# yanqinJiang/Animate3D

Measured on NVIDIA H100. Metric: MV-VDM denoise-steps/sec @ 4view x 16frame x 256^2, higher is better.
Workload: dtype fp16

## Files before the change

### animate3d_b200/csrc/a3d_attn.cu

```cuda
#include <stdlib.h>

#include <type_traits>

#include "a3d_common.cuh"
#include "a3d_host.cuh"
#include "a3d_wgmma.cuh"

namespace a3d {

struct AttnDev {
  int q_tiles, kv_tiles;
  int rows_q, rows_k;
  int heads;
  int q_t1, q_box1, q_box2, q_e1, q_e3;
  int k_t1, k_box1, k_box2, k_e3, kv_div, kv_i3_zero;
  uint32_t q_box_bytes, k_box_bytes;
  float scale_log2;
  __half* out;
  int64_t os1, os2, os3, os4;
  int accumulate;
  float out_scale;
  unsigned long long* dbg;
};

constexpr float kRescaleLog2 = 8.0f;
constexpr int kAttnThreads = 288;

template <int D>
struct AttnCfg {
  static constexpr int kDqk = (D + 15) / 16 * 16;
  static constexpr int kDv = (D + 1 + 15) / 16 * 16;
  static constexpr int kQB = (kDqk + 63) / 64;
  static constexpr int kVB = (kDv + 63) / 64;
  static constexpr int kStages = (D == 160) ? 3 : 4;
  static constexpr int kQBox = 128 * 128;
  static constexpr int kKVBox = 64 * 128;
  static constexpr int kSmemQ = kQB * kQBox;
  static constexpr int kSmemK = kStages * kQB * kKVBox;
  static constexpr int kSmemV = kStages * kVB * kKVBox;
  static constexpr int kSmemBytes = kSmemQ + kSmemK + kSmemV + 1024 + 256;
  static constexpr int kMinBlocks = (kSmemBytes <= 113 * 1024) ? 2 : 1;
  static_assert(kSmemBytes <= 227 * 1024, "shared memory budget");
};

template <int I, int N, class F>
__device__ __forceinline__ void static_for(F&& f) {
  if constexpr (I < N) {
    if (f(std::integral_constant<int, I>{})) static_for<I + 1, N>(f);
  }
}

template <int N>
__device__ __forceinline__ void wgmma_pv(float (&o)[N / 2], const uint32_t (&a)[4], uint64_t bdesc, uint32_t acc) {
  if constexpr (N == 48) wgmma_rs_n48<1>(o, a, bdesc, acc);
  else if constexpr (N == 96) wgmma_rs_n96<1>(o, a, bdesc, acc);
  else wgmma_rs_n176<1>(o, a, bdesc, acc);
}

template <int D>
__global__ void __launch_bounds__(kAttnThreads, AttnCfg<D>::kMinBlocks)
attn_tc_kernel(const AttnDev p, const __grid_constant__ CUtensorMap mapQ, const __grid_constant__ CUtensorMap mapK,
               const __grid_constant__ CUtensorMap mapV) {
  using Cfg = AttnCfg<D>;
  constexpr int S = Cfg::kStages;
  extern __shared__ uint8_t smem_raw[];
  uint8_t* smem = reinterpret_cast<uint8_t*>((reinterpret_cast<uintptr_t>(smem_raw) + 1023) & ~uintptr_t(1023));
  uint8_t* sQ = smem;
  uint8_t* sK = sQ + Cfg::kSmemQ;
  uint8_t* sV = sK + Cfg::kSmemK;
  uint64_t* bars = reinterpret_cast<uint64_t*>(sV + Cfg::kSmemV);
  uint64_t* q_full = bars;
  uint64_t* k_full = bars + 1;
  uint64_t* v_full = k_full + S;
  uint64_t* kv_empty = v_full + S;

  const int warp = threadIdx.x >> 5;
  const int lane = threadIdx.x & 31;
  const int qt = blockIdx.x;
  const int head = blockIdx.y;
  const int qb = blockIdx.z;
  const int n = p.kv_tiles;
  const int rows_tile = p.k_box1 * p.k_box2;

  if (p.rows_q < 128 || rows_tile < 64) {
    uint4* z = reinterpret_cast<uint4*>(sQ);
    const int n16 = (Cfg::kSmemQ + Cfg::kSmemK + Cfg::kSmemV) / 16;
    for (int i = threadIdx.x; i < n16; i += blockDim.x) z[i] = make_uint4(0, 0, 0, 0);
    fence_proxy_async_smem();
  }
  if (warp == 8 && lane == 0) {
    tma_prefetch_desc(&mapQ);
    tma_prefetch_desc(&mapK);
    tma_prefetch_desc(&mapV);
    mbar_init(q_full, 1);
    for (int i = 0; i < S; ++i) {
      mbar_init(&k_full[i], 1);
      mbar_init(&v_full[i], 1);
      mbar_init(&kv_empty[i], 8);
    }
    mbar_fence_init();
  }
  __syncthreads();

  const int q_i1 = (qt % p.q_t1) * p.q_box1;
  const int q_i2 = (qt / p.q_t1) * p.q_box2;
  const int q_i3 = qb % p.q_e3;
  const int q_i4 = qb / p.q_e3;

  if (warp == 8) {
    if (lane == 0) {
      const int kb = qb / p.kv_div;
      const int k_i3 = p.kv_i3_zero ? 0 : (kb % p.k_e3);
      const int k_i4 = kb / p.k_e3;
      mbar_expect_tx(q_full, p.q_box_bytes * Cfg::kQB);
#pragma unroll
      for (int b = 0; b < Cfg::kQB; ++b)
        tma_load_5d(sQ + b * Cfg::kQBox, &mapQ, q_full, head * Cfg::kDqk + b * 64, q_i1, q_i2, q_i3, q_i4);
      for (int j = 0; j < n; ++j) {
        const int st = j % S;
        const int k_i1 = (j % p.k_t1) * p.k_box1, k_i2 = (j / p.k_t1) * p.k_box2;
        mbar_wait(&kv_empty[st], ((j / S) & 1) ^ 1);
        mbar_expect_tx(&k_full[st], p.k_box_bytes * Cfg::kQB);
#pragma unroll
        for (int b = 0; b < Cfg::kQB; ++b)
          tma_load_5d(sK + (st * Cfg::kQB + b) * Cfg::kKVBox, &mapK, &k_full[st], head * Cfg::kDqk + b * 64, k_i1, k_i2, k_i3,
                      k_i4);
        mbar_expect_tx(&v_full[st], p.k_box_bytes * Cfg::kVB);
#pragma unroll
        for (int b = 0; b < Cfg::kVB; ++b)
          tma_load_5d(sV + (st * Cfg::kVB + b) * Cfg::kKVBox, &mapV, &v_full[st], head * Cfg::kDv + b * 64, k_i1, k_i2, k_i3,
                      k_i4);
      }
    }
    return;
  }

  const int wg = warp >> 2;
  const int g = lane >> 2, t = lane & 3;
  float s[32];
  float o[Cfg::kDv / 2];
#pragma unroll
  for (int i = 0; i < Cfg::kDv / 2; ++i) o[i] = 0.f;
  float m_lo = -INFINITY, m_hi = -INFINITY;
  const uint64_t qdesc = make_smem_desc_sw128(smem_u32(sQ + wg * (64 * 128)), 16, 1024);
  const uint64_t kdesc = make_smem_desc_sw128(smem_u32(sK), 16, 1024);
  const uint64_t vdesc = make_smem_desc_sw128(smem_u32(sV), Cfg::kKVBox, 1024);
  const int mask_from = rows_tile < 64 ? 0 : n - 1;
  uint32_t ph = 0;
  mbar_wait(q_full, 0);
  for (int j0 = 0; j0 < n; j0 += S) {
    static_for<0, S>([&](auto stc) {
      constexpr int st = decltype(stc)::value;
      const int j = j0 + st;
      if (j >= n) return false;
      mbar_wait(&k_full[st], ph);
      wgmma_fence();
#pragma unroll
      for (int kk = 0; kk < Cfg::kDqk / 16; ++kk)
        wgmma_ss_n64<0>(s, desc_add(qdesc, (kk / 4) * Cfg::kQBox + (kk % 4) * 32),
                        desc_add(kdesc, (st * Cfg::kQB + kk / 4) * Cfg::kKVBox + (kk % 4) * 32), kk ? 1u : 0u);
      wgmma_commit();
      wgmma_wait<0>();
      reg_fence(s);
      if (j >= mask_from) {
        const int valid = (j == n - 1) ? p.rows_k : rows_tile;
#pragma unroll
        for (int jj = 0; jj < 8; ++jj) {
#pragma unroll
          for (int e = 0; e < 2; ++e)
            if (8 * jj + 2 * t + e >= valid) { s[4 * jj + e] = -INFINITY; s[4 * jj + 2 + e] = -INFINITY; }
        }
      }
      float mx_lo = -INFINITY, mx_hi = -INFINITY;
#pragma unroll
      for (int jj = 0; jj < 8; ++jj) {
#pragma unroll
        for (int e = 0; e < 2; ++e) {
          mx_lo = fmaxf(mx_lo, s[4 * jj + e]);
          mx_hi = fmaxf(mx_hi, s[4 * jj + 2 + e]);
        }
      }
#pragma unroll
      for (int x = 1; x <= 2; x <<= 1) {
        mx_lo = fmaxf(mx_lo, __shfl_xor_sync(0xffffffffu, mx_lo, x));
        mx_hi = fmaxf(mx_hi, __shfl_xor_sync(0xffffffffu, mx_hi, x));
      }
      const float mn_lo = fmaxf(m_lo, mx_lo * p.scale_log2), mn_hi = fmaxf(m_hi, mx_hi * p.scale_log2);
      if (st == 0 && j == 0) {
        m_lo = mn_lo; m_hi = mn_hi;
      } else if (__any_sync(0xffffffffu, mn_lo - m_lo > kRescaleLog2 || mn_hi - m_hi > kRescaleLog2)) {
        if (p.dbg && lane == 0) atomicAdd(p.dbg, 1ull);
        const float a_lo = ex2_approx(m_lo - mn_lo), a_hi = ex2_approx(m_hi - mn_hi);
#pragma unroll
        for (int c = 0; c < Cfg::kDv / 8; ++c) {
          o[4 * c] *= a_lo; o[4 * c + 1] *= a_lo; o[4 * c + 2] *= a_hi; o[4 * c + 3] *= a_hi;
        }
        m_lo = mn_lo; m_hi = mn_hi;
      }
      uint32_t pa[4][4];
#pragma unroll
      for (int kk = 0; kk < 4; ++kk) {
#pragma unroll
        for (int h = 0; h < 2; ++h) {
          const float* sb = s + 4 * (2 * kk + h);
          pa[kk][2 * h] = pack_f16x2(ex2_approx(fmaf(sb[0], p.scale_log2, -m_lo)), ex2_approx(fmaf(sb[1], p.scale_log2, -m_lo)));
          pa[kk][2 * h + 1] = pack_f16x2(ex2_approx(fmaf(sb[2], p.scale_log2, -m_hi)), ex2_approx(fmaf(sb[3], p.scale_log2, -m_hi)));
        }
      }
      mbar_wait(&v_full[st], ph);
      wgmma_fence();
#pragma unroll
      for (int kk = 0; kk < 4; ++kk)
        wgmma_pv<Cfg::kDv>(o, pa[kk], desc_add(vdesc, st * Cfg::kVB * Cfg::kKVBox + kk * 2048), 1u);
      wgmma_commit();
      wgmma_wait<0>();
      reg_fence(o);
      __syncwarp();
      if (lane == 0) mbar_arrive(&kv_empty[st]);
      return true;
    });
    ph ^= 1;
  }
  const float l_lo = __shfl_sync(0xffffffffu, o[4 * (D / 8)], lane & ~3);
  const float l_hi = __shfl_sync(0xffffffffu, o[4 * (D / 8) + 2], lane & ~3);
#pragma unroll
  for (int h = 0; h < 2; ++h) {
    const int r = wg * 64 + (warp & 3) * 16 + g + 8 * h;
    const int i1 = q_i1 + r % p.q_box1;
    if (r >= p.rows_q || i1 >= p.q_e1) continue;
    const float inv = p.out_scale / (h ? l_hi : l_lo);
    const int i2 = q_i2 + r / p.q_box1;
    __half* orow = p.out + (int64_t)i1 * p.os1 + (int64_t)i2 * p.os2 + (int64_t)q_i3 * p.os3 + (int64_t)q_i4 * p.os4 +
                   head * D + 2 * t;
#pragma unroll
    for (int c = 0; c < D / 8; ++c) {
      float v0 = o[4 * c + 2 * h] * inv, v1 = o[4 * c + 2 * h + 1] * inv;
      if (p.accumulate) {
        const float2 f = __half22float2(*reinterpret_cast<const __half2*>(orow + 8 * c));
        v0 += f.x; v1 += f.y;
      }
      *reinterpret_cast<uint32_t*>(orow + 8 * c) = pack_f16x2(v0, v1);
    }
  }
}

struct ViewDev {
  const __half* base;
  int64_t s1, s2, s3, s4;
  int e1, e2, e3, e4;
};

constexpr int kFewKeysMax = 8;

template <int D>
__global__ void __launch_bounds__(256)
attn_fewkeys_kernel(ViewDev q, ViewDev k, ViewDev v, __half* out, int64_t os1, int64_t os2, int64_t os3, int64_t os4, int heads,
                    int dqk, int dv, float scale_log2, int kv_div, int kv_i3_zero, int accumulate, float out_scale) {
  constexpr int d = D;
  const int Lq = q.e1 * q.e2, Lk = k.e1 * k.e2;
  const int64_t total = (int64_t)q.e3 * q.e4 * Lq * heads;
  const int64_t idx = (int64_t)blockIdx.x * blockDim.x + threadIdx.x;
  if (idx >= total) return;
  const int h = (int)(idx % heads);
  const int64_t row = idx / heads;
  const int l = (int)(row % Lq);
  const int qb = (int)(row / Lq);
  const int kb = qb / kv_div;
  const __half* qp = q.base + (int64_t)(l % q.e1) * q.s1 + (int64_t)(l / q.e1) * q.s2 + (int64_t)(qb % q.e3) * q.s3 +
                     (int64_t)(qb / q.e3) * q.s4 + h * dqk;
  const int64_t koff = (int64_t)(kv_i3_zero ? 0 : kb % k.e3) * k.s3 + (int64_t)(kb / k.e3) * k.s4 + h * dqk;
  const int64_t voff = (int64_t)(kv_i3_zero ? 0 : kb % v.e3) * v.s3 + (int64_t)(kb / v.e3) * v.s4 + h * dv;
  int64_t krow[kFewKeysMax], vrow[kFewKeysMax];
#pragma unroll
  for (int j = 0; j < kFewKeysMax; ++j) {
    const int jj = j < Lk ? j : 0;
    krow[j] = koff + (int64_t)(jj % k.e1) * k.s1 + (int64_t)(jj / k.e1) * k.s2;
    vrow[j] = voff + (int64_t)(jj % v.e1) * v.s1 + (int64_t)(jj / v.e1) * v.s2;
  }
  float sc[kFewKeysMax];
#pragma unroll
  for (int j = 0; j < kFewKeysMax; ++j) sc[j] = 0.f;
#pragma unroll
  for (int c = 0; c < d; c += 8) {
    const uint4 qv = *reinterpret_cast<const uint4*>(qp + c);
    const __half2* qh = reinterpret_cast<const __half2*>(&qv);
    float2 qf[4];
#pragma unroll
    for (int t = 0; t < 4; ++t) qf[t] = __half22float2(qh[t]);
#pragma unroll
    for (int j = 0; j < kFewKeysMax; ++j) {
      if (j < Lk) {
        const uint4 kv = __ldg(reinterpret_cast<const uint4*>(k.base + krow[j] + c));
        const __half2* kh = reinterpret_cast<const __half2*>(&kv);
#pragma unroll
        for (int t = 0; t < 4; ++t) {
          const float2 kf = __half22float2(kh[t]);
          sc[j] = fmaf(qf[t].x, kf.x, fmaf(qf[t].y, kf.y, sc[j]));
        }
      }
    }
  }
  float m = -INFINITY;
#pragma unroll
  for (int j = 0; j < kFewKeysMax; ++j)
    if (j < Lk) m = fmaxf(m, sc[j]);
  float sum = 0.f;
#pragma unroll
  for (int j = 0; j < kFewKeysMax; ++j) {
    sc[j] = j < Lk ? exp2f((sc[j] - m) * scale_log2) : 0.f;
    sum += sc[j];
  }
  const float inv = out_scale / sum;
  __half* op = out + (int64_t)(l % q.e1) * os1 + (int64_t)(l / q.e1) * os2 + (int64_t)(qb % q.e3) * os3 +
               (int64_t)(qb / q.e3) * os4 + h * d;
#pragma unroll
  for (int c = 0; c < d; c += 8) {
    float acc[8];
#pragma unroll
    for (int t = 0; t < 8; ++t) acc[t] = 0.f;
#pragma unroll
    for (int j = 0; j < kFewKeysMax; ++j) {
      if (j < Lk) {
        const uint4 vv = __ldg(reinterpret_cast<const uint4*>(v.base + vrow[j] + c));
        const __half2* vh = reinterpret_cast<const __half2*>(&vv);
#pragma unroll
        for (int t = 0; t < 4; ++t) {
          const float2 vf = __half22float2(vh[t]);
          acc[2 * t] = fmaf(sc[j], vf.x, acc[2 * t]);
          acc[2 * t + 1] = fmaf(sc[j], vf.y, acc[2 * t + 1]);
        }
      }
    }
    uint4 o;
    __half2* oh = reinterpret_cast<__half2*>(&o);
    if (accumulate) {
      const uint4 old = *reinterpret_cast<const uint4*>(op + c);
      const __half2* ho = reinterpret_cast<const __half2*>(&old);
#pragma unroll
      for (int t = 0; t < 4; ++t) {
        const float2 f = __half22float2(ho[t]);
        oh[t] = __floats2half2_rn(fmaf(acc[2 * t], inv, f.x), fmaf(acc[2 * t + 1], inv, f.y));
      }
    } else {
#pragma unroll
      for (int t = 0; t < 4; ++t) oh[t] = __floats2half2_rn(acc[2 * t] * inv, acc[2 * t + 1] * inv);
    }
    *reinterpret_cast<uint4*>(op + c) = o;
  }
}

constexpr int kShortKeysPad = 80;
template <int D>
struct ShortCfg {
  static constexpr int kLdw = (D / 2 + 31) / 32 * 32 + 4;
  static constexpr int kLd = 2 * kLdw;
  static constexpr int kSmem = 2 * kShortKeysPad * kLd * 2;
};

template <int D>
__global__ void __launch_bounds__(128)
attn_shortkeys_kernel(ViewDev q, ViewDev k, ViewDev v, __half* out, int64_t os1, int64_t os2, int64_t os3, int64_t os4, int dqk,
                      int dv, float scale_log2, int kv_div, int kv_i3_zero, int accumulate, float out_scale, int rows_per_block) {
  using Cfg = ShortCfg<D>;
  constexpr int LD = Cfg::kLd;
  extern __shared__ __align__(16) uint8_t smraw[];
  __half* sK = reinterpret_cast<__half*>(smraw);
  __half* sV = sK + kShortKeysPad * LD;
  const int Lq = q.e1 * q.e2, Lk = k.e1 * k.e2;
  const int h = blockIdx.y, qb = blockIdx.z;
  const int kb = qb / kv_div;
  const int64_t koff = (int64_t)(kv_i3_zero ? 0 : kb % k.e3) * k.s3 + (int64_t)(kb / k.e3) * k.s4 + h * dqk;
  const int64_t voff = (int64_t)(kv_i3_zero ? 0 : kb % v.e3) * v.s3 + (int64_t)(kb / v.e3) * v.s4 + h * dv;
  constexpr int VPR = D / 8;
  for (int i = threadIdx.x; i < kShortKeysPad * VPR; i += blockDim.x) {
    const int j = i / VPR, c = i % VPR;
    uint4 kv4 = make_uint4(0, 0, 0, 0), vv4 = make_uint4(0, 0, 0, 0);
    if (j < Lk) {
      kv4 = __ldg(reinterpret_cast<const uint4*>(k.base + koff + (int64_t)(j % k.e1) * k.s1 + (int64_t)(j / k.e1) * k.s2) + c);
      vv4 = __ldg(reinterpret_cast<const uint4*>(v.base + voff + (int64_t)(j % v.e1) * v.s1 + (int64_t)(j / v.e1) * v.s2) + c);
    }
    *reinterpret_cast<uint4*>(sK + j * LD + c * 8) = kv4;
    *reinterpret_cast<uint4*>(sV + j * LD + c * 8) = vv4;
  }
  __syncthreads();
  const int warp = threadIdx.x >> 5, lane = threadIdx.x & 31;
  const int g = lane >> 2, t = lane & 3;
  const int row_begin = blockIdx.x * rows_per_block;
  const int row_end = min(row_begin + rows_per_block, Lq);
  const int64_t qbase = (int64_t)(qb % q.e3) * q.s3 + (int64_t)(qb / q.e3) * q.s4 + h * dqk;
  const int64_t obase = (int64_t)(qb % q.e3) * os3 + (int64_t)(qb / q.e3) * os4 + h * D;
  constexpr int KS = (D + 15) / 16;
  constexpr int NT = kShortKeysPad / 8;
  for (int r0 = row_begin + warp * 16; r0 < row_end; r0 += 64) {
    const int l_lo = r0 + g, l_hi = r0 + g + 8;
    const bool ok_lo = l_lo < row_end, ok_hi = l_hi < row_end;
    const __half* q_lo = q.base + qbase + (int64_t)(l_lo % q.e1) * q.s1 + (int64_t)(l_lo / q.e1) * q.s2;
    const __half* q_hi = q.base + qbase + (int64_t)(l_hi % q.e1) * q.s1 + (int64_t)(l_hi / q.e1) * q.s2;
    float s[NT][4];
#pragma unroll
    for (int nt = 0; nt < NT; ++nt) { s[nt][0] = 0.f; s[nt][1] = 0.f; s[nt][2] = 0.f; s[nt][3] = 0.f; }
#pragma unroll
    for (int kk = 0; kk < KS; ++kk) {
      const int d0 = kk * 16 + 2 * t;
      const bool hi_half = (kk * 16 + 8) < D;
      uint32_t a[4];
      a[0] = ok_lo ? __ldg(reinterpret_cast<const uint32_t*>(q_lo + d0)) : 0u;
      a[1] = ok_hi ? __ldg(reinterpret_cast<const uint32_t*>(q_hi + d0)) : 0u;
      a[2] = (ok_lo && hi_half) ? __ldg(reinterpret_cast<const uint32_t*>(q_lo + d0 + 8)) : 0u;
      a[3] = (ok_hi && hi_half) ? __ldg(reinterpret_cast<const uint32_t*>(q_hi + d0 + 8)) : 0u;
#pragma unroll
      for (int nt = 0; nt < NT; ++nt) {
        const __half* kr = sK + (nt * 8 + g) * LD + d0;
        const uint32_t b0 = *reinterpret_cast<const uint32_t*>(kr);
        const uint32_t b1 = hi_half ? *reinterpret_cast<const uint32_t*>(kr + 8) : 0u;
        mma_16816(s[nt], a, b0, b1);
      }
    }
    float mx_lo = -INFINITY, mx_hi = -INFINITY;
#pragma unroll
    for (int nt = 0; nt < NT; ++nt) {
      const int key = nt * 8 + 2 * t;
      if (key >= Lk) { s[nt][0] = -INFINITY; s[nt][2] = -INFINITY; }
      if (key + 1 >= Lk) { s[nt][1] = -INFINITY; s[nt][3] = -INFINITY; }
      mx_lo = fmaxf(mx_lo, fmaxf(s[nt][0], s[nt][1]));
      mx_hi = fmaxf(mx_hi, fmaxf(s[nt][2], s[nt][3]));
    }
#pragma unroll
    for (int o = 1; o <= 2; o <<= 1) {
      mx_lo = fmaxf(mx_lo, __shfl_xor_sync(0xffffffffu, mx_lo, o));
      mx_hi = fmaxf(mx_hi, __shfl_xor_sync(0xffffffffu, mx_hi, o));
    }
    const float nl = -mx_lo * scale_log2, nh = -mx_hi * scale_log2;
    float sum_lo = 0.f, sum_hi = 0.f;
#pragma unroll
    for (int nt = 0; nt < NT; ++nt) {
      s[nt][0] = ex2_approx(fmaf(s[nt][0], scale_log2, nl)); s[nt][1] = ex2_approx(fmaf(s[nt][1], scale_log2, nl));
      s[nt][2] = ex2_approx(fmaf(s[nt][2], scale_log2, nh)); s[nt][3] = ex2_approx(fmaf(s[nt][3], scale_log2, nh));
      sum_lo += s[nt][0] + s[nt][1];
      sum_hi += s[nt][2] + s[nt][3];
    }
#pragma unroll
    for (int o = 1; o <= 2; o <<= 1) {
      sum_lo += __shfl_xor_sync(0xffffffffu, sum_lo, o);
      sum_hi += __shfl_xor_sync(0xffffffffu, sum_hi, o);
    }
    const float inv_lo = 1.0f / sum_lo, inv_hi = 1.0f / sum_hi;
    uint32_t pa[NT / 2][4];
#pragma unroll
    for (int kk = 0; kk < NT / 2; ++kk) {
      pa[kk][0] = pack_f16x2(s[2 * kk][0] * inv_lo, s[2 * kk][1] * inv_lo);
      pa[kk][1] = pack_f16x2(s[2 * kk][2] * inv_hi, s[2 * kk][3] * inv_hi);
      pa[kk][2] = pack_f16x2(s[2 * kk + 1][0] * inv_lo, s[2 * kk + 1][1] * inv_lo);
      pa[kk][3] = pack_f16x2(s[2 * kk + 1][2] * inv_hi, s[2 * kk + 1][3] * inv_hi);
    }
    __half* o_lo = out + obase + (int64_t)(l_lo % q.e1) * os1 + (int64_t)(l_lo / q.e1) * os2;
    __half* o_hi = out + obase + (int64_t)(l_hi % q.e1) * os1 + (int64_t)(l_hi / q.e1) * os2;
#pragma unroll
    for (int nt = 0; nt < D / 8; ++nt) {
      float o[4] = {0.f, 0.f, 0.f, 0.f};
#pragma unroll
      for (int kk = 0; kk < NT / 2; ++kk) {
        const uint32_t addr = smem_u32(sV + (kk * 16 + (lane & 15)) * LD + nt * 8);
        uint32_t b0, b1;
        asm volatile("ldmatrix.sync.aligned.m8n8.x2.trans.shared.b16 {%0, %1}, [%2];" : "=r"(b0), "=r"(b1) : "r"(addr));
        mma_16816(o, pa[kk], b0, b1);
      }
      const int col = nt * 8 + 2 * t;
      if (ok_lo) {
        float x0 = o[0] * out_scale, x1 = o[1] * out_scale;
        if (accumulate) { const float2 f = __half22float2(*reinterpret_cast<const __half2*>(o_lo + col)); x0 += f.x; x1 += f.y; }
        *reinterpret_cast<uint32_t*>(o_lo + col) = pack_f16x2(x0, x1);
      }
      if (ok_hi) {
        float x0 = o[2] * out_scale, x1 = o[3] * out_scale;
        if (accumulate) { const float2 f = __half22float2(*reinterpret_cast<const __half2*>(o_hi + col)); x0 += f.x; x1 += f.y; }
        *reinterpret_cast<uint32_t*>(o_hi + col) = pack_f16x2(x0, x1);
      }
    }
  }
}

static ViewDev view_dev(const a3d_view5& v) {
  return ViewDev{reinterpret_cast<const __half*>(v.base), v.s1, v.s2, v.s3, v.s4, v.e1, v.e2, v.e3, v.e4};
}

static int tile_geom(const a3d_view5& v, int* box1, int* box2, int* t1, int* tiles, int* rows) {
  if (v.e1 >= 128) {
    if ((v.e1 % 128) && v.e2 != 1)
      return fail(A3D_EINVAL, "a3d_attention: inner extent %d is not a multiple of 128 and needs e2 == 1 (got %d)", v.e1, v.e2);
    *box1 = 128; *box2 = 1; *t1 = (v.e1 + 127) / 128; *tiles = *t1 * v.e2; *rows = 128;
  } else {
    int b2 = 128 / v.e1;
    if (b2 > v.e2) b2 = v.e2;
    if (b2 < 1 || v.e2 % b2) return fail(A3D_EINVAL, "a3d_attention: extents (%d,%d) do not tile", v.e1, v.e2);
    *box1 = v.e1; *box2 = b2; *t1 = 1; *tiles = v.e2 / b2; *rows = v.e1 * b2;
  }
  return 0;
}

static int view_map(const a3d_view5& v, int box1, int box2, const CUtensorMap** out) {
  const uint64_t dims[5] = {(uint64_t)v.cols, (uint64_t)v.e1, (uint64_t)v.e2, (uint64_t)v.e3, (uint64_t)v.e4};
  const uint64_t str[4] = {(uint64_t)v.s1, (uint64_t)v.s2, (uint64_t)v.s3, (uint64_t)v.s4};
  const uint32_t box[5] = {64, (uint32_t)box1, (uint32_t)box2, 1, 1};
  MapKey k = make_key(v.base, dims, str, box);
  return get_tensor_map(k, out);
}

static int tile_geom_k64(const a3d_view5& v, int* box1, int* box2, int* t1, int* tiles, int* rows_last) {
  if (v.e1 >= 64) {
    *box1 = 64; *box2 = 1; *t1 = (v.e1 + 63) / 64; *tiles = *t1 * v.e2;
    *rows_last = (v.e1 % 64) ? (v.e1 % 64) : 64;
    if ((v.e1 % 64) && v.e2 != 1) return fail(A3D_EINVAL, "a3d_attention: ragged key extent %d needs e2 == 1", v.e1);
  } else {
    int b2 = 64 / v.e1;
    if (b2 > v.e2) b2 = v.e2;
    if (b2 < 1 || v.e2 % b2) return fail(A3D_EINVAL, "a3d_attention: key extents (%d,%d) do not tile", v.e1, v.e2);
    *box1 = v.e1; *box2 = b2; *t1 = 1; *tiles = v.e2 / b2; *rows_last = v.e1 * b2;
  }
  return 0;
}

enum { kAttnFewKeys = 0, kAttnShortKeys = 1, kAttnTc = 2 };
static const char* const kAttnNames[] = {"fewkeys", "shortkeys", "tc"};

struct AttnPlan {
  int kernel;
  int dqk, dv, kv_div, batches;
  int qb1, qb2, qt1, qtiles, qrows;
  int kb1, kb2, kt1, ktiles, klast;
};

static int plan_attention(const a3d_attn_args* a, AttnPlan* p) {
  if (!a || !a->q.base || !a->k.base || !a->v.base || !a->out) return fail(A3D_EINVAL, "a3d_attention: null operand");
  const int d = a->d;
  if (d != 40 && d != 80 && d != 160) return fail(A3D_EINVAL, "a3d_attention: head dim %d not in {40,80,160}", d);
  if (a->k.e1 != a->v.e1 || a->k.e2 != a->v.e2 || a->k.e3 != a->v.e3 || a->k.e4 != a->v.e4)
    return fail(A3D_EINVAL, "a3d_attention: K and V extents differ");
  memset(p, 0, sizeof(*p));
  p->dqk = (d + 15) / 16 * 16;
  p->dv = (d + 1 + 15) / 16 * 16;
  p->kv_div = a->kv_div > 0 ? a->kv_div : 1;
  const int batches = p->batches = a->q.e3 * a->q.e4;
  if ((batches + p->kv_div - 1) / p->kv_div > a->k.e3 * a->k.e4 && !a->kv_i3_zero)
    return fail(A3D_EINVAL, "a3d_attention: key batches (%d) do not cover query batches (%d / %d)", a->k.e3 * a->k.e4,
                batches, p->kv_div);
  if (a->impl != A3D_GEMM_AUTO && a->impl != A3D_GEMM_TC)
    return fail(A3D_EINVAL, "a3d_attention: impl %d is not A3D_GEMM_AUTO or A3D_GEMM_TC", a->impl);
  if ((a->os1 | a->os2 | a->os3 | a->os4) % 8 || (reinterpret_cast<uintptr_t>(a->out) & 15))
    return fail(A3D_EINVAL, "a3d_attention: output rows must be 16-byte aligned");
  const bool auto_impl = a->impl == A3D_GEMM_AUTO;
  if (auto_impl && a->k.e1 * a->k.e2 <= kFewKeysMax) {
    if ((a->q.s1 | a->q.s2 | a->q.s3 | a->q.s4 | a->k.s1 | a->k.s2 | a->k.s3 | a->k.s4 | a->v.s1 | a->v.s2 | a->v.s3 | a->v.s4) % 8 ||
        ((reinterpret_cast<uintptr_t>(a->q.base) | reinterpret_cast<uintptr_t>(a->k.base) | reinterpret_cast<uintptr_t>(a->v.base)) & 15))
      return fail(A3D_EINVAL, "a3d_attention: operand rows must be 16-byte aligned");
    p->kernel = kAttnFewKeys;
    return A3D_OK;
  }
  if (auto_impl && a->k.e1 * a->k.e2 <= kShortKeysPad && (a->os1 | a->os2) % 2 == 0 &&
      ((a->k.s1 | a->k.s2 | a->k.s3 | a->k.s4 | a->v.s1 | a->v.s2 | a->v.s3 | a->v.s4) % 8 == 0) &&
      ((a->q.s1 | a->q.s2 | a->q.s3 | a->q.s4) % 2 == 0) &&
      ((reinterpret_cast<uintptr_t>(a->k.base) | reinterpret_cast<uintptr_t>(a->v.base)) & 15) == 0 &&
      (reinterpret_cast<uintptr_t>(a->q.base) & 3) == 0 && batches <= 65535) {
    p->kernel = kAttnShortKeys;
    return A3D_OK;
  }
  p->kernel = kAttnTc;
  if (int r = tile_geom(a->q, &p->qb1, &p->qb2, &p->qt1, &p->qtiles, &p->qrows)) return r;
  if (batches > 65535 || a->heads > 65535) return fail(A3D_EINVAL, "a3d_attention: grid too large");
  return tile_geom_k64(a->k, &p->kb1, &p->kb2, &p->kt1, &p->ktiles, &p->klast);
}

template <int D>
static int launch_fewkeys(const a3d_attn_args* a, const AttnPlan& p, cudaStream_t st) {
  const int64_t total = (int64_t)p.batches * a->heads * a->q.e1 * a->q.e2;
  attn_fewkeys_kernel<D><<<(unsigned)((total + 255) / 256), 256, 0, st>>>(
      view_dev(a->q), view_dev(a->k), view_dev(a->v), reinterpret_cast<__half*>(a->out), a->os1, a->os2, a->os3, a->os4,
      a->heads, p.dqk, p.dv, a->scale * 1.4426950408889634f, p.kv_div, a->kv_i3_zero, a->accumulate, a->out_scale);
  A3D_LAUNCH_CHECK();
  return A3D_OK;
}

template <int D>
static int launch_shortkeys(const a3d_attn_args* a, const AttnPlan& p, cudaStream_t st) {
  using Cfg = ShortCfg<D>;
  static bool attr_set = false;
  if (!attr_set && Cfg::kSmem > 48 * 1024) {
    A3D_CUDA_CHECK(cudaFuncSetAttribute(attn_shortkeys_kernel<D>, cudaFuncAttributeMaxDynamicSharedMemorySize, Cfg::kSmem));
    attr_set = true;
  }
  const int Lq = a->q.e1 * a->q.e2;
  int rows_per_block = 256;
  while (rows_per_block > 64 && (int64_t)((Lq + rows_per_block - 1) / rows_per_block) * a->heads * p.batches < 8 * sm_count())
    rows_per_block /= 2;
  dim3 grid((unsigned)((Lq + rows_per_block - 1) / rows_per_block), (unsigned)a->heads, (unsigned)p.batches);
  attn_shortkeys_kernel<D><<<grid, 128, Cfg::kSmem, st>>>(view_dev(a->q), view_dev(a->k), view_dev(a->v),
                                                          reinterpret_cast<__half*>(a->out), a->os1, a->os2, a->os3, a->os4,
                                                          p.dqk, p.dv, a->scale * 1.4426950408889634f, p.kv_div, a->kv_i3_zero,
                                                          a->accumulate, a->out_scale, rows_per_block);
  A3D_LAUNCH_CHECK();
  return A3D_OK;
}

static unsigned long long* g_attn_dbg = nullptr;

template <int D>
static int launch_attn(const a3d_attn_args* a, const AttnPlan& p, cudaStream_t st) {
  using Cfg = AttnCfg<D>;
  AttnDev dev;
  memset(&dev, 0, sizeof(dev));
  dev.q_tiles = p.qtiles; dev.rows_q = p.qrows;
  dev.kv_tiles = p.ktiles; dev.rows_k = p.klast;
  dev.heads = a->heads;
  dev.q_t1 = p.qt1; dev.q_box1 = p.qb1; dev.q_box2 = p.qb2; dev.q_e1 = a->q.e1; dev.q_e3 = a->q.e3;
  dev.k_t1 = p.kt1; dev.k_box1 = p.kb1; dev.k_box2 = p.kb2; dev.k_e3 = a->k.e3;
  dev.kv_div = p.kv_div; dev.kv_i3_zero = a->kv_i3_zero;
  dev.q_box_bytes = 128u * p.qrows;
  dev.k_box_bytes = 128u * (uint32_t)(p.kb1 * p.kb2);
  dev.scale_log2 = a->scale * 1.4426950408889634f;
  dev.out = reinterpret_cast<__half*>(a->out);
  dev.os1 = a->os1; dev.os2 = a->os2; dev.os3 = a->os3; dev.os4 = a->os4;
  dev.accumulate = a->accumulate;
  dev.out_scale = a->out_scale;
  dev.dbg = g_attn_dbg;
  const CUtensorMap *mq, *mk, *mv;
  if (int r = view_map(a->q, p.qb1, p.qb2, &mq)) return r;
  if (int r = view_map(a->k, p.kb1, p.kb2, &mk)) return r;
  if (int r = view_map(a->v, p.kb1, p.kb2, &mv)) return r;
  static bool attr_set = false;
  if (!attr_set) {
    A3D_CUDA_CHECK(cudaFuncSetAttribute(attn_tc_kernel<D>, cudaFuncAttributeMaxDynamicSharedMemorySize, Cfg::kSmemBytes));
    attr_set = true;
  }
  attn_tc_kernel<D><<<dim3(p.qtiles, a->heads, p.batches), kAttnThreads, Cfg::kSmemBytes, st>>>(dev, *mq, *mk, *mv);
  A3D_LAUNCH_CHECK();
  return A3D_OK;
}

template <int D>
static int launch_planned(const a3d_attn_args* a, const AttnPlan& p, cudaStream_t st) {
  switch (p.kernel) {
    case kAttnFewKeys: return launch_fewkeys<D>(a, p, st);
    case kAttnShortKeys: return launch_shortkeys<D>(a, p, st);
    default: return launch_attn<D>(a, p, st);
  }
}

}

extern "C" int a3d_attention_kernel(const a3d_attn_args* a, char* name, size_t n) {
  using namespace a3d;
  AttnPlan p;
  if (int r = plan_attention(a, &p)) return r;
  return kernel_name(name, n, "%s", kAttnNames[p.kernel]);
}

extern "C" int a3d_attention(const a3d_attn_args* a, void* stream) {
  using namespace a3d;
  cudaStream_t st = reinterpret_cast<cudaStream_t>(stream);
  AttnPlan p;
  if (int r = plan_attention(a, &p)) return r;
  switch (a->d) {
    case 40: return launch_planned<40>(a, p, st);
    case 80: return launch_planned<80>(a, p, st);
    default: return launch_planned<160>(a, p, st);
  }
}

extern "C" int a3d_debug_set_attn_trace(void* device_counter_u64) {
  a3d::g_attn_dbg = reinterpret_cast<unsigned long long*>(device_counter_u64);
  return A3D_OK;
}
```

### animate3d_b200/csrc/a3d_common.cuh

```cuda
#pragma once
#include <cuda.h>
#include <cuda_fp16.h>
#include <cuda_runtime.h>
#include <stdio.h>
#include <stdint.h>

namespace a3d {

__device__ __forceinline__ uint32_t smem_u32(const void* p) { return (uint32_t)__cvta_generic_to_shared(p); }

__device__ __forceinline__ void mbar_init(uint64_t* bar, uint32_t count) {
  asm volatile("mbarrier.init.shared::cta.b64 [%0], %1;" ::"r"(smem_u32(bar)), "r"(count) : "memory");
}
__device__ __forceinline__ void mbar_fence_init() { asm volatile("fence.mbarrier_init.release.cluster;" ::: "memory"); }

__device__ __forceinline__ void mbar_expect_tx(uint64_t* bar, uint32_t bytes) {
  asm volatile("mbarrier.arrive.expect_tx.shared::cta.b64 _, [%0], %1;" ::"r"(smem_u32(bar)), "r"(bytes) : "memory");
}
__device__ __forceinline__ void mbar_arrive(uint64_t* bar) {
  asm volatile("mbarrier.arrive.shared::cta.b64 _, [%0];" ::"r"(smem_u32(bar)) : "memory");
}
__device__ __forceinline__ bool mbar_try_wait(uint64_t* bar, uint32_t parity) {
  uint32_t ok;
  asm volatile(
      "{\n\t.reg .pred P;\n\t"
      "mbarrier.try_wait.parity.shared::cta.b64 P, [%1], %2;\n\t"
      "selp.b32 %0, 1, 0, P;\n\t}\n"
      : "=r"(ok)
      : "r"(smem_u32(bar)), "r"(parity)
      : "memory");
  return ok != 0;
}
__device__ __forceinline__ void mbar_wait(uint64_t* bar, uint32_t parity) {
  if (mbar_try_wait(bar, parity)) return;
  const long long t0 = clock64();
  while (!mbar_try_wait(bar, parity)) {
    if (clock64() - t0 > 8000000000ll) __trap();
  }
}

__device__ __forceinline__ void tma_prefetch_desc(const CUtensorMap* m) {
  asm volatile("prefetch.tensormap [%0];" ::"l"(reinterpret_cast<uint64_t>(m)) : "memory");
}
__device__ __forceinline__ void tma_load_5d(void* smem_dst, const CUtensorMap* map, uint64_t* bar, int c0, int c1, int c2,
                                            int c3, int c4) {
  asm volatile(
      "cp.async.bulk.tensor.5d.shared::cluster.global.mbarrier::complete_tx::bytes"
      " [%0], [%1, {%3, %4, %5, %6, %7}], [%2];"
      :
      : "r"(smem_u32(smem_dst)), "l"(reinterpret_cast<uint64_t>(map)), "r"(smem_u32(bar)), "r"(c0), "r"(c1), "r"(c2),
        "r"(c3), "r"(c4)
      : "memory");
}
__device__ __forceinline__ void fence_proxy_async_smem() { asm volatile("fence.proxy.async.shared::cta;" ::: "memory"); }

__device__ __forceinline__ void st_global_256(void* ptr, const uint32_t* r) {
  asm volatile("st.global.v4.b32 [%0], {%1, %2, %3, %4};" ::"l"(ptr), "r"(r[0]), "r"(r[1]), "r"(r[2]), "r"(r[3]) : "memory");
  asm volatile("st.global.v4.b32 [%0], {%1, %2, %3, %4};" ::"l"(reinterpret_cast<uint8_t*>(ptr) + 16), "r"(r[4]), "r"(r[5]),
               "r"(r[6]), "r"(r[7])
               : "memory");
}

__device__ __forceinline__ float ex2_approx(float x) {
  float y;
  asm("ex2.approx.ftz.f32 %0, %1;" : "=f"(y) : "f"(x));
  return y;
}
__device__ __forceinline__ uint32_t pack_f16x2(float lo, float hi) {
  uint32_t d;
  asm("cvt.rn.f16x2.f32 %0, %1, %2;" : "=r"(d) : "f"(hi), "f"(lo));
  return d;
}
__device__ __forceinline__ void wgmma_fence() { asm volatile("wgmma.fence.sync.aligned;" ::: "memory"); }
__device__ __forceinline__ void wgmma_commit() { asm volatile("wgmma.commit_group.sync.aligned;" ::: "memory"); }
template <int N>
__device__ __forceinline__ void wgmma_wait() { asm volatile("wgmma.wait_group.sync.aligned %0;" ::"n"(N) : "memory"); }
template <int R>
__device__ __forceinline__ void reg_fence(float (&d)[R]) {
#pragma unroll
  for (int i = 0; i < R; ++i) asm volatile("" : "+f"(d[i])::"memory");
}
__device__ __forceinline__ uint64_t make_smem_desc_sw128(uint32_t smem_addr, uint32_t lbo_bytes, uint32_t sbo_bytes) {
  uint64_t d = 0;
  d |= (uint64_t)((smem_addr >> 4) & 0x3FFF);
  d |= (uint64_t)((lbo_bytes >> 4) & 0x3FFF) << 16;
  d |= (uint64_t)((sbo_bytes >> 4) & 0x3FFF) << 32;
  d |= (uint64_t)1 << 62;
  return d;
}
__device__ __forceinline__ uint64_t desc_add(uint64_t desc, uint32_t bytes) {
  return (desc & 0xFFFFFFFF00000000ull) | (uint32_t)((uint32_t)desc + (bytes >> 4));
}

__device__ __forceinline__ void mma_16816(float (&c)[4], const uint32_t (&a)[4], uint32_t b0, uint32_t b1) {
  asm volatile("mma.sync.aligned.m16n8k16.row.col.f32.f16.f16.f32 {%0,%1,%2,%3}, {%4,%5,%6,%7}, {%8,%9}, {%0,%1,%2,%3};"
               : "+f"(c[0]), "+f"(c[1]), "+f"(c[2]), "+f"(c[3])
               : "r"(a[0]), "r"(a[1]), "r"(a[2]), "r"(a[3]), "r"(b0), "r"(b1));
}

}
```

Before: 6.591.

## Make tensor-core attention persistent with warp-specialized producer and double-buffered Q

Replaces the one-CTA-per-tile attention kernel (for head dims other than 40) with a persistent kernel launched at SM count that loops over tiles. A dedicated producer warpgroup drops its register budget via setmaxnreg and streams Q (double-buffered when shared memory allows) and K/V through mbarriers, while two consumer warpgroups raise theirs. The aim is to hide per-tile prologue, Q load latency and launch tail, and to give the consumers more registers. The old kernel stays as a pair kernel for D=40. Risks: one CTA per SM with a large shared-memory footprint, and load imbalance across tiles.

```diff
diff --git a/animate3d_b200/csrc/a3d_attn.cu b/animate3d_b200/csrc/a3d_attn.cu
--- a/animate3d_b200/csrc/a3d_attn.cu
+++ b/animate3d_b200/csrc/a3d_attn.cu
@@ -9,6 +9,7 @@
 namespace a3d {
 
 struct AttnDev {
+  int tiles;
   int q_tiles, kv_tiles;
   int rows_q, rows_k;
   int heads;
@@ -24,10 +25,312 @@
 };
 
 constexpr float kRescaleLog2 = 8.0f;
-constexpr int kAttnThreads = 288;
+constexpr int kAttnThreads = 384;
 
 template <int D>
 struct AttnCfg {
+  static constexpr int kDqk = (D + 15) / 16 * 16;
+  static constexpr int kDv = (D + 1 + 15) / 16 * 16;
+  static constexpr int kQB = (kDqk + 63) / 64;
+  static constexpr int kVB = (kDv + 63) / 64;
+  static constexpr int kStages = (D == 160) ? 3 : 4;
+  static constexpr int kQBox = 128 * 128;
+  static constexpr int kKVBox = 64 * 128;
+  static constexpr int kSmemQ = kQB * kQBox;
+  static constexpr int kSmemK = kStages * kQB * kKVBox;
+  static constexpr int kSmemV = kStages * kVB * kKVBox;
+  static constexpr int kSmemRest = kSmemK + kSmemV + 1024 + 256;
+  static constexpr int kQBufs = (2 * kSmemQ + kSmemRest <= 227 * 1024) ? 2 : 1;
+  static constexpr int kSmemBytes = kQBufs * kSmemQ + kSmemRest;
+  static_assert(kSmemBytes <= 227 * 1024, "shared memory budget");
+};
+
+template <int I, int N, class F>
+__device__ __forceinline__ void static_for(F&& f) {
+  if constexpr (I < N) {
+    if (f(std::integral_constant<int, I>{})) static_for<I + 1, N>(f);
+  }
+}
+
+template <int N>
+__device__ __forceinline__ void wgmma_pv(float (&o)[N / 2], const uint32_t (&a)[4], uint64_t bdesc, uint32_t acc) {
+  if constexpr (N == 48) wgmma_rs_n48<1>(o, a, bdesc, acc);
+  else if constexpr (N == 96) wgmma_rs_n96<1>(o, a, bdesc, acc);
+  else wgmma_rs_n176<1>(o, a, bdesc, acc);
+}
+
+template <int D>
+__global__ void __launch_bounds__(kAttnThreads, 1)
+attn_tc_kernel(const AttnDev p, const __grid_constant__ CUtensorMap mapQ, const __grid_constant__ CUtensorMap mapK,
+               const __grid_constant__ CUtensorMap mapV) {
+  using Cfg = AttnCfg<D>;
+  constexpr int S = Cfg::kStages;
+  constexpr int QN = Cfg::kQBufs;
+  extern __shared__ uint8_t smem_raw[];
+  uint8_t* smem = reinterpret_cast<uint8_t*>((reinterpret_cast<uintptr_t>(smem_raw) + 1023) & ~uintptr_t(1023));
+  uint8_t* sQ = smem;
+  uint8_t* sK = sQ + QN * Cfg::kSmemQ;
+  uint8_t* sV = sK + Cfg::kSmemK;
+  uint64_t* bars = reinterpret_cast<uint64_t*>(sV + Cfg::kSmemV);
+  uint64_t* q_full = bars;
+  uint64_t* q_empty = q_full + QN;
+  uint64_t* k_full = q_empty + QN;
+  uint64_t* v_full = k_full + S;
+  uint64_t* kv_empty = v_full + S;
+
+  const int warp = threadIdx.x >> 5;
+  const int lane = threadIdx.x & 31;
+  const int n = p.kv_tiles;
+  const int rows_tile = p.k_box1 * p.k_box2;
+
+  if (p.rows_q < 128 || rows_tile < 64) {
+    uint4* z = reinterpret_cast<uint4*>(sQ);
+    const int n16 = (QN * Cfg::kSmemQ + Cfg::kSmemK + Cfg::kSmemV) / 16;
+    for (int i = threadIdx.x; i < n16; i += blockDim.x) z[i] = make_uint4(0, 0, 0, 0);
+    fence_proxy_async_smem();
+  }
+  if (threadIdx.x == 0) {
+    tma_prefetch_desc(&mapQ);
+    tma_prefetch_desc(&mapK);
+    tma_prefetch_desc(&mapV);
+    for (int i = 0; i < QN; ++i) {
+      mbar_init(&q_full[i], 1);
+      mbar_init(&q_empty[i], 8);
+    }
+    for (int i = 0; i < S; ++i) {
+      mbar_init(&k_full[i], 1);
+      mbar_init(&v_full[i], 1);
+      mbar_init(&kv_empty[i], 8);
+    }
+    mbar_fence_init();
+  }
+  __syncthreads();
+
+  if (warp < 4) {
+    setmaxnreg_dec<32>();
+    if (warp == 0 && lane == 0) {
+      uint32_t eph = 0;
+      int it = 0;
+      for (int tile = blockIdx.x; tile < p.tiles; tile += gridDim.x, ++it) {
+        const int qt = tile % p.q_tiles, hq = tile / p.q_tiles;
+        const int head = hq % p.heads, qb = hq / p.heads;
+        const int qs = it % QN;
+        mbar_wait(&q_empty[qs], ((it / QN) & 1) ^ 1);
+        mbar_expect_tx(&q_full[qs], p.q_box_bytes * Cfg::kQB);
+#pragma unroll
+        for (int b = 0; b < Cfg::kQB; ++b)
+          tma_load_5d(sQ + qs * Cfg::kSmemQ + b * Cfg::kQBox, &mapQ, &q_full[qs], head * Cfg::kDqk + b * 64,
+                      (qt % p.q_t1) * p.q_box1, (qt / p.q_t1) * p.q_box2, qb % p.q_e3, qb / p.q_e3);
+        const int kb = qb / p.kv_div;
+        const int k_i3 = p.kv_i3_zero ? 0 : (kb % p.k_e3);
+        const int k_i4 = kb / p.k_e3;
+        for (int j = 0; j < n; ++j) {
+          const int st = j % S;
+          const int k_i1 = (j % p.k_t1) * p.k_box1, k_i2 = (j / p.k_t1) * p.k_box2;
+          mbar_wait(&kv_empty[st], ((eph >> st) & 1) ^ 1);
+          eph ^= 1u << st;
+          mbar_expect_tx(&k_full[st], p.k_box_bytes * Cfg::kQB);
+#pragma unroll
+          for (int b = 0; b < Cfg::kQB; ++b)
+            tma_load_5d(sK + (st * Cfg::kQB + b) * Cfg::kKVBox, &mapK, &k_full[st], head * Cfg::kDqk + b * 64, k_i1, k_i2,
+                        k_i3, k_i4);
+          mbar_expect_tx(&v_full[st], p.k_box_bytes * Cfg::kVB);
+#pragma unroll
+          for (int b = 0; b < Cfg::kVB; ++b)
+            tma_load_5d(sV + (st * Cfg::kVB + b) * Cfg::kKVBox, &mapV, &v_full[st], head * Cfg::kDv + b * 64, k_i1, k_i2,
+                        k_i3, k_i4);
+        }
+      }
+      for (int st = 0; st < S; ++st) mbar_wait(&kv_empty[st], ((eph >> st) & 1) ^ 1);
+    }
+    return;
+  }
+
+  setmaxnreg_inc<232>();
+  const int wg = (warp >> 2) - 1;
+  const int g = lane >> 2, t = lane & 3;
+  constexpr int U = (S % 2) ? 2 * S : S;
+  float s[2][32];
+  uint32_t pa[4][4];
+  float o[Cfg::kDv / 2];
+  float m_lo, m_hi;
+  uint32_t kph = 0, vph = 0;
+  const uint64_t kdesc = make_smem_desc_sw128(smem_u32(sK), 16, 1024);
+  const uint64_t vdesc = make_smem_desc_sw128(smem_u32(sV), Cfg::kKVBox, 1024);
+
+  auto softmax = [&](float (&sc)[32], bool first, bool mask, int valid, float& m_old_lo, float& m_old_hi) {
+    if (mask) {
+#pragma unroll
+      for (int jj = 0; jj < 8; ++jj) {
+#pragma unroll
+        for (int e = 0; e < 2; ++e)
+          if (8 * jj + 2 * t + e >= valid) { sc[4 * jj + e] = -INFINITY; sc[4 * jj + 2 + e] = -INFINITY; }
+      }
+    }
+    float mx_lo = -INFINITY, mx_hi = -INFINITY;
+#pragma unroll
+    for (int jj = 0; jj < 8; ++jj) {
+#pragma unroll
+      for (int e = 0; e < 2; ++e) {
+        mx_lo = fmaxf(mx_lo, sc[4 * jj + e]);
+        mx_hi = fmaxf(mx_hi, sc[4 * jj + 2 + e]);
+      }
+    }
+#pragma unroll
+    for (int x = 1; x <= 2; x <<= 1) {
+      mx_lo = fmaxf(mx_lo, __shfl_xor_sync(0xffffffffu, mx_lo, x));
+      mx_hi = fmaxf(mx_hi, __shfl_xor_sync(0xffffffffu, mx_hi, x));
+    }
+    const float mn_lo = fmaxf(m_lo, mx_lo * p.scale_log2), mn_hi = fmaxf(m_hi, mx_hi * p.scale_log2);
+    const bool rescale = !first && __any_sync(0xffffffffu, mn_lo - m_lo > kRescaleLog2 || mn_hi - m_hi > kRescaleLog2);
+    m_old_lo = m_lo; m_old_hi = m_hi;
+    if (first || rescale) { m_lo = mn_lo; m_hi = mn_hi; }
+#pragma unroll
+    for (int i = 0; i < 32; i += 4) {
+      sc[i] = ex2_approx(fmaf(sc[i], p.scale_log2, -m_lo)); sc[i + 1] = ex2_approx(fmaf(sc[i + 1], p.scale_log2, -m_lo));
+      sc[i + 2] = ex2_approx(fmaf(sc[i + 2], p.scale_log2, -m_hi)); sc[i + 3] = ex2_approx(fmaf(sc[i + 3], p.scale_log2, -m_hi));
+    }
+    return rescale;
+  };
+  auto issue_qk = [&](float (&sd)[32], uint64_t qdesc, int st) {
+    uint64_t kd = kdesc;
+    asm volatile("" : "+l"(kd), "+l"(qdesc));
+#pragma unroll
+    for (int kk = 0; kk < Cfg::kDqk / 16; ++kk)
+      wgmma_ss_n64<0>(sd, desc_add(qdesc, (kk / 4) * Cfg::kQBox + (kk % 4) * 32),
+                      desc_add(kd, (st * Cfg::kQB + kk / 4) * Cfg::kKVBox + (kk % 4) * 32), kk ? 1u : 0u);
+    wgmma_commit();
+  };
+  auto issue_pv = [&](int st) {
+    uint64_t vd = vdesc;
+    asm volatile("" : "+l"(vd));
+#pragma unroll
+    for (int kk = 0; kk < 4; ++kk)
+      wgmma_pv<Cfg::kDv>(o, pa[kk], desc_add(vd, st * Cfg::kVB * Cfg::kKVBox + kk * 2048), 1u);
+    wgmma_commit();
+  };
+  auto wait_k = [&](int st) { mbar_spin(&k_full[st], (kph >> st) & 1); kph ^= 1u << st; };
+  auto wait_v = [&](int st) { mbar_spin(&v_full[st], (vph >> st) & 1); vph ^= 1u << st; };
+  auto release = [&](uint64_t* bar) { __syncwarp(); if (lane == 0) mbar_arrive(bar); };
+
+  auto step = [&](float (&sc)[32], float (&sn)[32], uint64_t qdesc, uint64_t* q_rel, int j, int st_next, int st_prev,
+                  bool has_next, bool has_prev, bool mask, int valid) {
+    if (has_next || has_prev) {
+      if (has_next) wait_k(st_next);
+      if (has_prev) wait_v(st_prev);
+      wgmma_fence();
+      if (has_next) issue_qk(sn, qdesc, st_next);
+      if (has_prev) issue_pv(st_prev);
+    }
+    float m_old_lo, m_old_hi;
+    const bool rescale = softmax(sc, !has_prev, mask, valid, m_old_lo, m_old_hi);
+    reg_fence(sc);
+    if (has_next || has_prev) {
+      wgmma_wait<0>();
+      reg_fence(o);
+      reg_fence(sc);
+      if (has_next) reg_fence(sn);
+      if (has_prev) release(&kv_empty[st_prev]);
+      if (has_next && j + 1 == n - 1) release(q_rel);
+    }
+    if (rescale) {
+      if (p.dbg && lane == 0) atomicAdd(p.dbg, 1ull);
+      const float a_lo = ex2_approx(m_old_lo - m_lo), a_hi = ex2_approx(m_old_hi - m_hi);
+#pragma unroll
+      for (int c = 0; c < Cfg::kDv / 8; ++c) {
+        o[4 * c] *= a_lo; o[4 * c + 1] *= a_lo; o[4 * c + 2] *= a_hi; o[4 * c + 3] *= a_hi;
+      }
+    }
+#pragma unroll
+    for (int kk = 0; kk < 4; ++kk) {
+#pragma unroll
+      for (int h = 0; h < 2; ++h) {
+        const float* sb = sc + 4 * (2 * kk + h);
+        pa[kk][2 * h] = pack_f16x2(sb[0], sb[1]);
+        pa[kk][2 * h + 1] = pack_f16x2(sb[2], sb[3]);
+      }
+    }
+  };
+
+  int it = 0;
+  for (int tile = blockIdx.x; tile < p.tiles; tile += gridDim.x, ++it) {
+    const int qt = tile % p.q_tiles, hq = tile / p.q_tiles;
+    const int head = hq % p.heads, qb = hq / p.heads;
+    const int qs = it % QN;
+    const uint64_t qdesc = make_smem_desc_sw128(smem_u32(sQ + qs * Cfg::kSmemQ + wg * (64 * 128)), 16, 1024);
+#pragma unroll
+    for (int i = 0; i < Cfg::kDv / 2; ++i) o[i] = 0.f;
+    m_lo = -INFINITY; m_hi = -INFINITY;
+    mbar_spin(&q_full[qs], (it / QN) & 1);
+    wait_k(0);
+    wgmma_fence();
+    issue_qk(s[0], qdesc, 0);
+    wgmma_wait<0>();
+    reg_fence(s[0]);
+    if (n == 1) {
+      release(&q_empty[qs]);
+      step(s[0], s[1], qdesc, &q_empty[qs], 0, 0, 0, false, false, true, p.rows_k);
+    } else {
+      auto steps = [&](auto mask_all) {
+        step(s[0], s[1], qdesc, &q_empty[qs], 0, 1 % S, 0, true, false, mask_all, rows_tile);
+        for (int j0 = 0; j0 < n - 1; j0 += U) {
+          static_for<0, U>([&](auto ic) {
+            constexpr int i = decltype(ic)::value;
+            const int j = j0 + i;
+            if (i == 0 && j == 0) return true;
+            if (j >= n - 1) return false;
+            step(s[i & 1], s[(i + 1) & 1], qdesc, &q_empty[qs], j, (i + 1) % S, (i + S - 1) % S, true, true, mask_all,
+                 rows_tile);
+            return true;
+          });
+        }
+      };
+      if (rows_tile < 64) steps(std::true_type{});
+      else steps(std::false_type{});
+      if ((n - 1) & 1) step(s[1], s[0], qdesc, &q_empty[qs], n - 1, 0, (n - 2) % S, false, true, true, p.rows_k);
+      else step(s[0], s[1], qdesc, &q_empty[qs], n - 1, 0, (n - 2) % S, false, true, true, p.rows_k);
+    }
+    {
+      const int st = (n - 1) % S;
+      wait_v(st);
+      wgmma_fence();
+      issue_pv(st);
+      wgmma_wait<0>();
+      reg_fence(o);
+      release(&kv_empty[st]);
+    }
+    const int q_i1 = (qt % p.q_t1) * p.q_box1;
+    const int q_i2 = (qt / p.q_t1) * p.q_box2;
+    const int q_i3 = qb % p.q_e3;
+    const int q_i4 = qb / p.q_e3;
+    const float l_lo = __shfl_sync(0xffffffffu, o[4 * (D / 8)], lane & ~3);
+    const float l_hi = __shfl_sync(0xffffffffu, o[4 * (D / 8) + 2], lane & ~3);
+#pragma unroll
+    for (int h = 0; h < 2; ++h) {
+      const int r = wg * 64 + (warp & 3) * 16 + g + 8 * h;
+      const int i1 = q_i1 + r % p.q_box1;
+      if (r >= p.rows_q || i1 >= p.q_e1) continue;
+      const float inv = p.out_scale / (h ? l_hi : l_lo);
+      const int i2 = q_i2 + r / p.q_box1;
+      __half* orow = p.out + (int64_t)i1 * p.os1 + (int64_t)i2 * p.os2 + (int64_t)q_i3 * p.os3 + (int64_t)q_i4 * p.os4 +
+                     head * D + 2 * t;
+#pragma unroll
+      for (int c = 0; c < D / 8; ++c) {
+        float v0 = o[4 * c + 2 * h] * inv, v1 = o[4 * c + 2 * h + 1] * inv;
+        if (p.accumulate) {
+          const float2 f = __half22float2(*reinterpret_cast<const __half2*>(orow + 8 * c));
+          v0 += f.x; v1 += f.y;
+        }
+        *reinterpret_cast<uint32_t*>(orow + 8 * c) = pack_f16x2(v0, v1);
+      }
+    }
+  }
+}
+
+constexpr int kAttnPairThreads = 288;
+
+template <int D>
+struct AttnPairCfg {
   static constexpr int kDqk = (D + 15) / 16 * 16;
   static constexpr int kDv = (D + 1 + 15) / 16 * 16;
   static constexpr int kQB = (kDqk + 63) / 64;
@@ -43,25 +346,11 @@
   static_assert(kSmemBytes <= 227 * 1024, "shared memory budget");
 };
 
-template <int I, int N, class F>
-__device__ __forceinline__ void static_for(F&& f) {
-  if constexpr (I < N) {
-    if (f(std::integral_constant<int, I>{})) static_for<I + 1, N>(f);
-  }
-}
-
-template <int N>
-__device__ __forceinline__ void wgmma_pv(float (&o)[N / 2], const uint32_t (&a)[4], uint64_t bdesc, uint32_t acc) {
-  if constexpr (N == 48) wgmma_rs_n48<1>(o, a, bdesc, acc);
-  else if constexpr (N == 96) wgmma_rs_n96<1>(o, a, bdesc, acc);
-  else wgmma_rs_n176<1>(o, a, bdesc, acc);
-}
-
-template <int D>
-__global__ void __launch_bounds__(kAttnThreads, AttnCfg<D>::kMinBlocks)
-attn_tc_kernel(const AttnDev p, const __grid_constant__ CUtensorMap mapQ, const __grid_constant__ CUtensorMap mapK,
+template <int D>
+__global__ void __launch_bounds__(kAttnPairThreads, AttnPairCfg<D>::kMinBlocks)
+attn_tc_pair_kernel(const AttnDev p, const __grid_constant__ CUtensorMap mapQ, const __grid_constant__ CUtensorMap mapK,
                const __grid_constant__ CUtensorMap mapV) {
-  using Cfg = AttnCfg<D>;
+  using Cfg = AttnPairCfg<D>;
   constexpr int S = Cfg::kStages;
   extern __shared__ uint8_t smem_raw[];
   uint8_t* smem = reinterpret_cast<uint8_t*>((reinterpret_cast<uintptr_t>(smem_raw) + 1023) & ~uintptr_t(1023));
@@ -566,7 +855,8 @@
   }
   p->kernel = kAttnTc;
   if (int r = tile_geom(a->q, &p->qb1, &p->qb2, &p->qt1, &p->qtiles, &p->qrows)) return r;
-  if (batches > 65535 || a->heads > 65535) return fail(A3D_EINVAL, "a3d_attention: grid too large");
+  if (batches > 65535 || a->heads > 65535 || (int64_t)p->qtiles * a->heads * batches > INT32_MAX)
+    return fail(A3D_EINVAL, "a3d_attention: grid too large");
   return tile_geom_k64(a->k, &p->kb1, &p->kb2, &p->kt1, &p->ktiles, &p->klast);
 }
 
@@ -608,6 +898,7 @@
   using Cfg = AttnCfg<D>;
   AttnDev dev;
   memset(&dev, 0, sizeof(dev));
+  dev.tiles = p.qtiles * a->heads * p.batches;
   dev.q_tiles = p.qtiles; dev.rows_q = p.qrows;
   dev.kv_tiles = p.ktiles; dev.rows_k = p.klast;
   dev.heads = a->heads;
@@ -627,11 +918,21 @@
   if (int r = view_map(a->k, p.kb1, p.kb2, &mk)) return r;
   if (int r = view_map(a->v, p.kb1, p.kb2, &mv)) return r;
   static bool attr_set = false;
-  if (!attr_set) {
-    A3D_CUDA_CHECK(cudaFuncSetAttribute(attn_tc_kernel<D>, cudaFuncAttributeMaxDynamicSharedMemorySize, Cfg::kSmemBytes));
-    attr_set = true;
-  }
-  attn_tc_kernel<D><<<dim3(p.qtiles, a->heads, p.batches), kAttnThreads, Cfg::kSmemBytes, st>>>(dev, *mq, *mk, *mv);
+  if constexpr (D == 40) {
+    using PCfg = AttnPairCfg<D>;
+    if (!attr_set) {
+      A3D_CUDA_CHECK(cudaFuncSetAttribute(attn_tc_pair_kernel<D>, cudaFuncAttributeMaxDynamicSharedMemorySize, PCfg::kSmemBytes));
+      attr_set = true;
+    }
+    attn_tc_pair_kernel<D><<<dim3(p.qtiles, a->heads, p.batches), kAttnPairThreads, PCfg::kSmemBytes, st>>>(dev, *mq, *mk, *mv);
+  } else {
+    if (!attr_set) {
+      A3D_CUDA_CHECK(cudaFuncSetAttribute(attn_tc_kernel<D>, cudaFuncAttributeMaxDynamicSharedMemorySize, Cfg::kSmemBytes));
+      attr_set = true;
+    }
+    const int grid = dev.tiles < sm_count() ? dev.tiles : sm_count();
+    attn_tc_kernel<D><<<grid, kAttnThreads, Cfg::kSmemBytes, st>>>(dev, *mq, *mk, *mv);
+  }
   A3D_LAUNCH_CHECK();
   return A3D_OK;
 }
diff --git a/animate3d_b200/csrc/a3d_common.cuh b/animate3d_b200/csrc/a3d_common.cuh
--- a/animate3d_b200/csrc/a3d_common.cuh
+++ b/animate3d_b200/csrc/a3d_common.cuh
@@ -36,6 +36,16 @@
   const long long t0 = clock64();
   while (!mbar_try_wait(bar, parity)) {
     if (clock64() - t0 > 8000000000ll) __trap();
+  }
+}
+
+template <int R>
+__device__ __forceinline__ void setmaxnreg_dec() { asm volatile("setmaxnreg.dec.sync.aligned.u32 %0;" ::"n"(R)); }
+template <int R>
+__device__ __forceinline__ void setmaxnreg_inc() { asm volatile("setmaxnreg.inc.sync.aligned.u32 %0;" ::"n"(R)); }
+
+__device__ __forceinline__ void mbar_spin(uint64_t* bar, uint32_t parity) {
+  while (!mbar_try_wait(bar, parity)) {
   }
 }
 
```

Result: no change. 6.602 (median of 6 runs) (+0.2%).
